# yangfei1223/CRFConv

Measured on AMD Instinct MI355X. Metric: M points/sec fwd+bwd, S3DIS 40960-pt cloud, K=16, 3 CRF iters; mIoU parity, higher is better.
Workload: dtype f32; 1 GPU; BASELINE configs[1]: S3DIS-like synthetic clouds (one point per 4 cm voxel of an 8x8x3 m box), 4 clouds x 40960 pts per GPU, K=16, ratios [4,4,4,4,2], PointConvBig(in=6, classes=13, use_crf, steps=3), train mode: fwd + weighted CE + bwd + flat-bucket grad all-reduce + SGD(momentum) step; tables resident in HBM; point order from the device collate: morton; global_batch=4, points_per_cloud=40960, parallelism=dp1 (batch-sharded)

## Files before the change

### crfconv_amd/csrc/pointconv_wide.hip

```cpp
#include "common.hpp"
#include "gridsync.hpp"

namespace crf {

using f32x4w = __attribute__((ext_vector_type(4))) float;
#ifndef WP_BLOCK_
#define WP_BLOCK_ 512
#endif
constexpr int WP_BLOCK = WP_BLOCK_, WP_WAVES = WP_BLOCK / WAVE, WP_MAX = 8;

struct WideJobs {
    const float* x[WP_MAX]; const float* gout[WP_MAX]; const float* pos_src[WP_MAX]; const float* pos_tgt[WP_MAX];
    const int32_t* idx[WP_MAX];
    const float* A1[WP_MAX]; const float* b1[WP_MAX]; const float* W2[WP_MAX]; const float* ca[WP_MAX]; const float* cb[WP_MAX];
    const float* cc[WP_MAX];
    float* dw2_partial[WP_MAX]; double* a1_partial[WP_MAX];
    int m_tgt[WP_MAX], nblk[WP_MAX], d[WP_MAX];
    float slope[WP_MAX];
    int blk_base[WP_MAX + 1];
    int njobs;
};

template <int D>
constexpr int wide_params_lds_floats() {
    return D * (D + 4) + 4 * D + 3 * D + WP_WAVES * 16 * (D + 4) + WP_WAVES * 16 * (D + 16) + 4 * WP_WAVES * 16;
}
template <int D>
__device__ __forceinline__ void wide_params_body(const WideJobs& t, const int job, const int blk, float* __restrict__ lds) {
    constexpr int T16 = D / 16, S4 = D / 4, LDW = D + 4, LDG = D + 4, LDH = D + 16, K = 16;
    constexpr int UNR = S4 > 16 ? 4 : S4;
    float* const s_w2 = lds;
    float4* const s_a1 = reinterpret_cast<float4*>(s_w2 + D * LDW);
    float* const s_coef = reinterpret_cast<float*>(s_a1 + D);
    float (*s_g)[K * LDG] = reinterpret_cast<float (*)[K * LDG]>(s_coef + 3 * D);
    float (*s_h)[K * LDH] = reinterpret_cast<float (*)[K * LDH]>(s_coef + 3 * D + WP_WAVES * K * LDG);
    float4 (*s_rel)[K] = reinterpret_cast<float4 (*)[K]>(s_coef + 3 * D + WP_WAVES * K * (LDG + LDH));
    float* s_red = s_w2;
    const int nblk = t.nblk[job], m = t.m_tgt[job];
    const float* __restrict__ x = t.x[job];
    const float* __restrict__ gout = t.gout[job];
    const float* __restrict__ pos_src = t.pos_src[job];
    const float* __restrict__ pos_tgt = t.pos_tgt[job];
    const int32_t* __restrict__ idx = t.idx[job];
    const float slope = t.slope[job];
    {
        const float* __restrict__ W2 = t.W2[job];
        for (int i = threadIdx.x; i < D * D; i += WP_BLOCK) s_w2[(i / D) * LDW + (i % D)] = W2[i];
        const float* __restrict__ A1 = t.A1[job];
        const float* __restrict__ b1 = t.b1[job];
        for (int c = threadIdx.x; c < D; c += WP_BLOCK) {
            s_a1[c] = make_float4(A1[3 * c], A1[3 * c + 1], A1[3 * c + 2], b1[c]);
            s_coef[c] = t.ca[job][c];
            s_coef[D + c] = t.cb[job][c];
            s_coef[2 * D + c] = t.cc[job][c];
        }
    }
    __syncthreads();
    const int lane = threadIdx.x & 63, wave = threadIdx.x >> 6;
    const int e = lane & 15, kq = lane >> 4;
    float* tg = s_g[wave];
    float* th = s_h[wave];
    float4* trel = s_rel[wave];
    f32x4w accW[T16][T16];
#pragma unroll
    for (int a = 0; a < T16; ++a)
#pragma unroll
        for (int b = 0; b < T16; ++b) accW[a][b] = f32x4w{0.f, 0.f, 0.f, 0.f};
    float a1acc[T16][4];
#pragma unroll
    for (int a = 0; a < T16; ++a)
#pragma unroll
        for (int b = 0; b < 4; ++b) a1acc[a][b] = 0.f;

    const int per = (m + nblk - 1) / nblk;
    const int p0 = blk * per, p1 = p0 + per < m ? p0 + per : m;
    for (int p = p0 + wave; p < p1; p += WP_WAVES) {
        const int jraw = idx[(int64_t)p * K + e];
        const bool live = jraw >= 0;
        const int64_t j = live ? jraw : 0;
        const float rx = pos_tgt[3 * (int64_t)p] - pos_src[3 * j], ry = pos_tgt[3 * (int64_t)p + 1] - pos_src[3 * j + 1],
                    rz = pos_tgt[3 * (int64_t)p + 2] - pos_src[3 * j + 2];
        int jr[4];
        bool lr[4];
#pragma unroll
        for (int r = 0; r < 4; ++r) {
            jr[r] = __shfl((int)j, 4 * kq + r, WAVE);
            lr[r] = __shfl(live ? 1 : 0, 4 * kq + r, WAVE) != 0;
        }
        constexpr bool PRELOAD = D <= 64;
        [[maybe_unused]] float xv[PRELOAD ? T16 : 1][4], gi[PRELOAD ? T16 : 1];
        if constexpr (PRELOAD) {
#pragma unroll
            for (int tj = 0; tj < T16; ++tj) {
                gi[tj] = gout[(int64_t)p * D + 16 * tj + e];
#pragma unroll
                for (int r = 0; r < 4; ++r) xv[tj][r] = x[(int64_t)jr[r] * D + 16 * tj + e];
            }
        }
        if (kq == 0) trel[e] = live ? make_float4(rx, ry, rz, 1.f) : make_float4(0.f, 0.f, 0.f, 0.f);
        f32x4w acc[T16];
#pragma unroll
        for (int tj = 0; tj < T16; ++tj) acc[tj] = f32x4w{0.f, 0.f, 0.f, 0.f};
#pragma unroll UNR
        for (int s = 0; s < S4; ++s) {
            const float4 a = s_a1[4 * s + kq];
            const float pre = fmaf(a.x, rx, fmaf(a.y, ry, fmaf(a.z, rz, a.w)));
            const float h = live ? (pre > 0.f ? pre : slope * pre) : 0.f;
            th[e * LDH + 4 * s + kq] = h;
#pragma unroll
            for (int tj = 0; tj < T16; ++tj)
                acc[tj] = __builtin_amdgcn_mfma_f32_16x16x4f32(h, s_w2[(16 * tj + e) * LDW + 4 * s + kq], acc[tj], 0, 0, 0);
        }
#pragma unroll
        for (int tj = 0; tj < T16; ++tj) {
            const int c = 16 * tj + e;
            const float va = s_coef[c], vb = s_coef[D + c], vc = s_coef[2 * D + c];
            float gic, xc[4];
            if constexpr (PRELOAD) {
                gic = gi[tj];
#pragma unroll
                for (int r = 0; r < 4; ++r) xc[r] = xv[tj][r];
            } else {
                gic = gout[(int64_t)p * D + c];
#pragma unroll
                for (int r = 0; r < 4; ++r) xc[r] = x[(int64_t)jr[r] * D + c];
            }
#pragma unroll
            for (int r = 0; r < 4; ++r) {
                const float gh = fmaf(va, gic * xc[r], fmaf(vb, acc[tj][r], vc));
                tg[(4 * kq + r) * LDG + c] = lr[r] ? gh : 0.f;
            }
        }
        __builtin_amdgcn_wave_barrier();
#pragma unroll
        for (int tj = 0; tj < T16; ++tj) acc[tj] = f32x4w{0.f, 0.f, 0.f, 0.f};
#pragma unroll UNR
        for (int s = 0; s < S4; ++s) {
            const float a = tg[e * LDG + 4 * s + kq];
#pragma unroll
            for (int tj = 0; tj < T16; ++tj)
                acc[tj] = __builtin_amdgcn_mfma_f32_16x16x4f32(a, s_w2[(4 * s + kq) * LDW + 16 * tj + e], acc[tj], 0, 0, 0);
        }
        {
            float4 rl[4];
#pragma unroll
            for (int r = 0; r < 4; ++r) rl[r] = trel[4 * kq + r];
#pragma unroll
            for (int tj = 0; tj < T16; ++tj)
#pragma unroll
                for (int r = 0; r < 4; ++r) {
                    const float h = th[(4 * kq + r) * LDH + 16 * tj + e];
                    const float gp = acc[tj][r] * (h > 0.f ? 1.f : slope);
                    a1acc[tj][0] = fmaf(gp, rl[r].x, a1acc[tj][0]);
                    a1acc[tj][1] = fmaf(gp, rl[r].y, a1acc[tj][1]);
                    a1acc[tj][2] = fmaf(gp, rl[r].z, a1acc[tj][2]);
                    a1acc[tj][3] = fmaf(gp, rl[r].w, a1acc[tj][3]);
                }
        }
#pragma unroll
        for (int s = 0; s < 4; ++s) {
            float af[T16], bf[T16];
#pragma unroll
            for (int ti = 0; ti < T16; ++ti) {
                af[ti] = tg[(4 * s + kq) * LDG + 16 * ti + e];
                bf[ti] = th[(4 * s + kq) * LDH + 16 * ti + e];
            }
#pragma unroll
            for (int ti = 0; ti < T16; ++ti)
#pragma unroll
                for (int tj = 0; tj < T16; ++tj)
                    accW[ti][tj] = __builtin_amdgcn_mfma_f32_16x16x4f32(af[ti], bf[tj], accW[ti][tj], 0, 0, 0);
        }
        __builtin_amdgcn_wave_barrier();
    }
    __syncthreads();
    for (int w = 0; w < WP_WAVES; ++w) {
        if (wave == w) {
#pragma unroll
            for (int ti = 0; ti < T16; ++ti)
#pragma unroll
                for (int tj = 0; tj < T16; ++tj)
#pragma unroll
                    for (int r = 0; r < 4; ++r) {
                        const int o = (16 * ti + 4 * kq + r) * D + 16 * tj + e;
                        s_red[o] = (w == 0 ? 0.f : s_red[o]) + accW[ti][tj][r];
                    }
        }
        __syncthreads();
    }
    {
        float* __restrict__ out = t.dw2_partial[job] + (int64_t)blk * D * D;
        for (int i = threadIdx.x; i < D * D; i += WP_BLOCK) out[i] = s_red[i];
    }
    __syncthreads();
#pragma unroll
    for (int tj = 0; tj < T16; ++tj)
#pragma unroll
        for (int q = 0; q < 4; ++q) {
            float v = a1acc[tj][q];
            v += __shfl_xor(v, 16, WAVE);
            v += __shfl_xor(v, 32, WAVE);
            if (kq == 0) s_red[(wave * D + 16 * tj + e) * 4 + q] = v;
        }
    __syncthreads();
    {
        double* __restrict__ outd = t.a1_partial[job] + (int64_t)blk * 4 * D;
        for (int i = threadIdx.x; i < 4 * D; i += WP_BLOCK) {
            double a = 0.0;
#pragma unroll
            for (int w = 0; w < WP_WAVES; ++w) a += (double)s_red[w * 4 * D + i];
            outd[i] = a;
        }
    }
}

__global__ __launch_bounds__(WP_BLOCK) void wide_params_any_kernel(const WideJobs t) {
    __shared__ __attribute__((aligned(16))) float lds[wide_params_lds_floats<64>()];
    int job = 0;
    while (job + 1 < t.njobs && t.blk_base[job + 1] <= (int)blockIdx.x) ++job;
    const int blk = (int)blockIdx.x - t.blk_base[job];
    if (t.d[job] == 32) wide_params_body<32>(t, job, blk, lds);
    else wide_params_body<64>(t, job, blk, lds);
}

template <int D>
__global__ __launch_bounds__(WP_BLOCK) void uvstats_mfma_kernel(const float* __restrict__ x, const float* __restrict__ pos_src,
                                                                const float* __restrict__ pos_tgt, const int32_t* __restrict__ idx,
                                                                int m, int nblk, const float* __restrict__ A1,
                                                                const float* __restrict__ b1, const float* __restrict__ W2, float slope,
                                                                const float* __restrict__ mean_rel, float* __restrict__ shift_out,
                                                                float* __restrict__ U, float* __restrict__ V, float* __restrict__ partial,
                                                                unsigned* __restrict__ ticket, double* __restrict__ stats) {
    constexpr int T16 = D / 16, S4 = D / 4, LDW = D + 4, K = 16;
    constexpr int UNR = S4 > 16 ? 4 : S4;
    __shared__ __attribute__((aligned(16))) float s_w2[D * LDW];
    __shared__ float4 s_a1[D];
    __shared__ float s_shift[D];
    __shared__ float s_h0[D];
    __shared__ float s_red[WP_WAVES][2][D];
    for (int i = threadIdx.x; i < D * D; i += WP_BLOCK) s_w2[(i / D) * LDW + (i % D)] = W2[i];
    for (int c = threadIdx.x; c < D; c += WP_BLOCK) {
        const float4 a = make_float4(A1[3 * c], A1[3 * c + 1], A1[3 * c + 2], b1[c]);
        s_a1[c] = a;
        const float pre = fmaf(a.x, mean_rel[0], fmaf(a.y, mean_rel[1], fmaf(a.z, mean_rel[2], a.w)));
        s_h0[c] = pre > 0.f ? pre : slope * pre;
    }
    __syncthreads();
    for (int c = threadIdx.x; c < D; c += WP_BLOCK) {
        float a = 0.f;
        for (int cp = 0; cp < D; ++cp) a = fmaf(s_h0[cp], s_w2[c * LDW + cp], a);
        s_shift[c] = a;
        if (blockIdx.x == 0) shift_out[c] = a;
    }
    __syncthreads();
    const int lane = threadIdx.x & 63, wave = threadIdx.x >> 6;
    const int e = lane & 15, kq = lane >> 4;
    float st1[T16], st2[T16];
#pragma unroll
    for (int tj = 0; tj < T16; ++tj) st1[tj] = st2[tj] = 0.f;
    const int per = (m + nblk - 1) / nblk;
    const int p0 = (int)blockIdx.x * per, p1 = p0 + per < m ? p0 + per : m;
    for (int p = p0 + wave; p < p1; p += WP_WAVES) {
        const int jraw = idx[(int64_t)p * K + e];
        const bool live = jraw >= 0;
        const int64_t j = live ? jraw : 0;
        const float rx = pos_tgt[3 * (int64_t)p] - pos_src[3 * j], ry = pos_tgt[3 * (int64_t)p + 1] - pos_src[3 * j + 1],
                    rz = pos_tgt[3 * (int64_t)p + 2] - pos_src[3 * j + 2];
        int jr[4];
        float lv[4];
#pragma unroll
        for (int r = 0; r < 4; ++r) {
            jr[r] = __shfl((int)j, 4 * kq + r, WAVE);
            lv[r] = __shfl(live ? 1.f : 0.f, 4 * kq + r, WAVE);
        }
        float xv[T16][4];
#pragma unroll
        for (int tj = 0; tj < T16; ++tj)
#pragma unroll
            for (int r = 0; r < 4; ++r) xv[tj][r] = x[(int64_t)jr[r] * D + 16 * tj + e] * lv[r];
        f32x4w acc[T16];
#pragma unroll
        for (int tj = 0; tj < T16; ++tj) acc[tj] = f32x4w{0.f, 0.f, 0.f, 0.f};
#pragma unroll UNR
        for (int s = 0; s < S4; ++s) {
            const float4 a = s_a1[4 * s + kq];
            const float pre = fmaf(a.x, rx, fmaf(a.y, ry, fmaf(a.z, rz, a.w)));
            const float h = pre > 0.f ? pre : slope * pre;
#pragma unroll
            for (int tj = 0; tj < T16; ++tj)
                acc[tj] = __builtin_amdgcn_mfma_f32_16x16x4f32(h, s_w2[(16 * tj + e) * LDW + 4 * s + kq], acc[tj], 0, 0, 0);
        }
#pragma unroll
        for (int tj = 0; tj < T16; ++tj) {
            const float sh = s_shift[16 * tj + e];
            float u = 0.f, v = 0.f;
#pragma unroll
            for (int r = 0; r < 4; ++r) {
                const float dlt = (acc[tj][r] - sh) * lv[r];
                st1[tj] += dlt;
                st2[tj] = fmaf(dlt, dlt, st2[tj]);
                u = fmaf(dlt, xv[tj][r], u);
                v += xv[tj][r];
            }
            u += __shfl_xor(u, 16, WAVE); u += __shfl_xor(u, 32, WAVE);
            v += __shfl_xor(v, 16, WAVE); v += __shfl_xor(v, 32, WAVE);
            if (kq == 0) {
                U[(int64_t)p * D + 16 * tj + e] = u;
                V[(int64_t)p * D + 16 * tj + e] = v;
            }
        }
    }
#pragma unroll
    for (int tj = 0; tj < T16; ++tj) {
        float a = st1[tj], b = st2[tj];
        a += __shfl_xor(a, 16, WAVE); a += __shfl_xor(a, 32, WAVE);
        b += __shfl_xor(b, 16, WAVE); b += __shfl_xor(b, 32, WAVE);
        if (kq == 0) { s_red[wave][0][16 * tj + e] = a; s_red[wave][1][16 * tj + e] = b; }
    }
    __syncthreads();
    const __amdgpu_buffer_rsrc_t pr = make_rsrc(partial, (int)gridDim.x * 2 * D * 4);
    for (int i = threadIdx.x; i < 2 * D; i += WP_BLOCK) {
        float a = 0.f;
#pragma unroll
        for (int w = 0; w < WP_WAVES; ++w) a += s_red[w][i / D][i % D];
        st1_sc1(pr, ((int)blockIdx.x * 2 * D + i) * 4, a);
    }
    constexpr bool ALIAS = sizeof(float) * D * LDW >= sizeof(double) * 4 * WP_BLOCK;
    __shared__ double s_own[ALIAS ? 1 : 4 * WP_BLOCK], s_tot[2 * D];
    __shared__ int s_flag;
    if (ticket == nullptr || !last_workgroup(ticket, gridDim.x, &s_flag)) return;
    double* s_buf = ALIAS ? reinterpret_cast<double*>(s_w2) : s_own;
    sum_partial_rows_f64<WP_BLOCK>(pr, (int)gridDim.x, 2 * D, s_buf, s_tot);
    if (threadIdx.x < 2 * D) stats[threadIdx.x] = s_tot[threadIdx.x];
}

#ifndef WP_PPW_BIG_
#define WP_PPW_BIG_ 3
#endif
#ifndef WP_PPW_MID_
#define WP_PPW_MID_ 3
#endif
#ifndef WP_PPW_SMALL_
#define WP_PPW_SMALL_ 1
#endif
static int64_t wide_points_per_wave(int64_t m_tgt) {
    return m_tgt >= 8192 ? WP_PPW_BIG_ : (m_tgt >= 2048 ? WP_PPW_MID_ : WP_PPW_SMALL_);
}

bool uvstats_mfma_ok(int K, int d) { return K == 16 && (d == 32 || d == 64 || d == 128); }
int uvstats_mfma_launch(const float* x, const float* pos_src, const float* pos_tgt, const int32_t* idx32, int64_t m_tgt, int d,
                        const float* A1, const float* b1, const float* W2, float slope, const float* mean_rel3, float* shift, float* U,
                        float* V, float* partial, int64_t max_blocks, int64_t* nblk_out, unsigned* ticket, double* stats, hipStream_t st) {
    int64_t nb = cdiv(m_tgt, wide_points_per_wave(m_tgt) * WP_WAVES);
    if (nb > max_blocks) nb = max_blocks;
    if (nb < 1) nb = 1;
    *nblk_out = nb;
    if (d == 32) hipLaunchKernelGGL(uvstats_mfma_kernel<32>, dim3((unsigned)nb), dim3(WP_BLOCK), 0, st, x, pos_src, pos_tgt, idx32, (int)m_tgt, (int)nb, A1, b1, W2, slope, mean_rel3, shift, U, V, partial, ticket, stats);
    else if (d == 64) hipLaunchKernelGGL(uvstats_mfma_kernel<64>, dim3((unsigned)nb), dim3(WP_BLOCK), 0, st, x, pos_src, pos_tgt, idx32, (int)m_tgt, (int)nb, A1, b1, W2, slope, mean_rel3, shift, U, V, partial, ticket, stats);
    else hipLaunchKernelGGL(uvstats_mfma_kernel<128>, dim3((unsigned)nb), dim3(WP_BLOCK), 0, st, x, pos_src, pos_tgt, idx32, (int)m_tgt, (int)nb, A1, b1, W2, slope, mean_rel3, shift, U, V, partial, ticket, stats);
    CRF_LAUNCH_CHECK();
    return CRF_OK;
}

static int64_t wide_nblk(int64_t m_tgt, int d) {
    (void)d;
    int64_t nb = cdiv(m_tgt, wide_points_per_wave(m_tgt) * WP_WAVES);
    if (nb < 1) nb = 1;
    if (nb > 2048) nb = 2048;
    return nb;
}

}

using namespace crf;

extern "C" int crfconv_pointconv_wide_params_supported(int64_t m_tgt, int K, int d) {
    return (K == 16 && (d == 32 || d == 64) && m_tgt > 0 && m_tgt < ((int64_t)1 << 27)) ? 1 : 0;
}

extern "C" int64_t crfconv_pointconv_wide_params_nblk(int64_t m_tgt, int d) {
    return m_tgt > 0 ? wide_nblk(m_tgt, d) : 0;
}

extern "C" int crfconv_pointconv_wide_params_jobs(const crf_pc_wide_job* jobs, int njobs, crf_stream_t stream) {
    CRF_REQUIRE(jobs || njobs == 0, CRF_ERR_ARG, "null pointer");
    CRF_REQUIRE(njobs >= 0, CRF_ERR_ARG, "njobs=%d < 0", njobs);
    hipStream_t st = as_stream(stream);
    for (int j = 0; j < njobs; ++j) {
        const crf_pc_wide_job& jb = jobs[j];
        CRF_REQUIRE(crfconv_pointconv_wide_params_supported(jb.m_tgt, jb.K, jb.d) == 1, CRF_ERR_UNSUPPORTED,
                    "job %d: K=%d d=%d m_tgt=%lld outside the matrix-pipe parameter pass (K = 16, d in {32, 64})", j, jb.K, jb.d,
                    (long long)jb.m_tgt);
        CRF_REQUIRE(jb.x && jb.gout && jb.pos_src && jb.pos_tgt && jb.idx32 && jb.A1 && jb.b1 && jb.W2 && jb.ca && jb.cb && jb.cc &&
                        jb.dw2_partial && jb.a1_partial, CRF_ERR_ARG, "job %d: null pointer", j);
    }
    int order[2] = {64, 32};
    int idx[64];
    int nidx = 0;
    for (int w = 0; w < 2; ++w)
        for (int j = 0; j < njobs && nidx < 64; ++j)
            if (jobs[j].d == order[w]) idx[nidx++] = j;
    CRF_REQUIRE(nidx == njobs, CRF_ERR_UNSUPPORTED, "at most 64 jobs per call");
    for (int j0 = 0; j0 < nidx; j0 += WP_MAX) {
        WideJobs t;
        const int n = nidx - j0 < WP_MAX ? nidx - j0 : WP_MAX;
        int64_t blocks = 0;
        for (int k = 0; k < n; ++k) {
            const crf_pc_wide_job& jb = jobs[idx[j0 + k]];
            t.x[k] = jb.x; t.gout[k] = jb.gout; t.pos_src[k] = jb.pos_src; t.pos_tgt[k] = jb.pos_tgt; t.idx[k] = jb.idx32;
            t.A1[k] = jb.A1; t.b1[k] = jb.b1; t.W2[k] = jb.W2; t.ca[k] = jb.ca; t.cb[k] = jb.cb; t.cc[k] = jb.cc;
            t.dw2_partial[k] = jb.dw2_partial; t.a1_partial[k] = jb.a1_partial;
            t.m_tgt[k] = (int)jb.m_tgt; t.nblk[k] = (int)wide_nblk(jb.m_tgt, jb.d); t.slope[k] = jb.slope; t.d[k] = jb.d;
            t.blk_base[k] = (int)blocks;
            blocks += t.nblk[k];
        }
        for (int k = n; k <= WP_MAX; ++k) t.blk_base[k] = (int)blocks;
        for (int k = n; k < WP_MAX; ++k) {
            t.x[k] = t.gout[k] = t.pos_src[k] = t.pos_tgt[k] = t.A1[k] = t.b1[k] = t.W2[k] = t.ca[k] = t.cb[k] = t.cc[k] = nullptr;
            t.idx[k] = nullptr; t.dw2_partial[k] = nullptr; t.a1_partial[k] = nullptr; t.m_tgt[k] = 0; t.nblk[k] = 1; t.slope[k] = 1.f; t.d[k] = 32;
        }
        t.njobs = n;
        hipLaunchKernelGGL(wide_params_any_kernel, dim3((unsigned)blocks), dim3(WP_BLOCK), 0, st, t);
        CRF_LAUNCH_CHECK();
    }
    return CRF_OK;
}
```

### crfconv_amd/ops/_base.py

```python
import ctypes

import torch

from .. import _lib
from ..graph import NeighborTable, ptr, require_gpu, stream_ptr

BN_EPS = 1e-5


def _f32c(t):
    if t.dtype is torch.float32 and t.is_contiguous():
        return t.detach()
    return t.detach().to(torch.float32).contiguous()


def _pad_channels(t, C):
    if t.shape[-1] == C:
        return t
    return torch.nn.functional.pad(t, (0, C - t.shape[-1]))


def _next_supported(c, choices):
    for v in choices:
        if c <= v:
            return v
    raise _lib.CrfConvError('channel count %d exceeds the largest supported (%d)' % (c, choices[-1]))


def _ptr_array(tensors):
    return (ctypes.c_void_p * len(tensors))(*[None if t is None else t.data_ptr() for t in tensors])



_TICKETS = {}
_raw_stream = getattr(torch._C, '_cuda_getCurrentRawStream', None)


def _stream_key(device):
    idx = device.index if isinstance(device, torch.device) else None
    if idx is None:
        dev = torch.device(device)
        idx = dev.index if dev.index is not None else torch.cuda.current_device()
    if torch.cuda.is_current_stream_capturing():
        return idx, 'capture'
    if _raw_stream is not None:
        return idx, int(_raw_stream(idx))
    return idx, int(torch.cuda.current_stream(idx).cuda_stream)


def _stream_buf(table, device, make):
    key = _stream_key(device)
    buf = table.get(key)
    if buf is None:
        buf = table[key] = make()
        if key[1] != 'capture' and (key[0], 'capture') not in table:
            table[(key[0], 'capture')] = make()
    return buf


def _ticket(device):
    return _stream_buf(_TICKETS, device, lambda: torch.zeros(_lib.load().crfconv_ticket_bytes() // 4, dtype=torch.int32, device=device))




def _pc_ticket(device):
    return ptr(_ticket(device))




def _mlp_ticket(device):
    return ptr(_ticket(device))


_sync_ws = {}


def gridsync_ws(dev):
    return _stream_buf(_sync_ws, dev, lambda: torch.zeros(_lib.load().crfconv_gridsync_workspace() // 4, dtype=torch.int32, device=dev))




def fail_word_ptrs(dev):
    want = torch.device(dev).index
    if want is None:
        want = torch.cuda.current_device()
    word = _lib.load().crfconv_gridsync_fail_word()
    keys = [k for k in _sync_ws if k[0] == want]
    first = [k for k in ((want, 'capture'), (want, int(torch.cuda.current_stream(want).cuda_stream))) if k in _sync_ws]
    rest = [k for k in reversed(keys) if k not in first]
    if len(first) + len(rest) > 8:
        import warnings
        warnings.warn('fail_word_ptrs: %d barrier workspaces on device %d, the update guard watches 8 (capture buffer, current stream, '
                      'newest streams); ops.check_gridsync() reads all of them' % (len(first) + len(rest), want))
    return [_sync_ws[k].data_ptr() + 4 * word for k in (first + rest)[:8]]


def check_gridsync(dev=None, reduced_flag=None):
    word = _lib.load().crfconv_gridsync_fail_word()
    bad = []
    want = None if dev is None else torch.device(dev).index
    for table in (_sync_ws,):
        for key, ws in list(table.items()):
            if want is not None and key[0] is not None and key[0] != want:
                continue
            code = int(ws[word].item())
            if code != 0:
                ws.zero_()
                bad.append((key, code))
    remote = False
    if reduced_flag is not None and reduced_flag.numel():
        v = float(reduced_flag.reshape(-1)[0].item())
        remote = not (v == 0.0)
        if remote:
            reduced_flag.zero_()
    if bad or remote:
        state.small_mlp_disabled = True
        where = ('device(s) %s (code 0x%x)' % (sorted({k[0] for k, _ in bad}), bad[0][1])) if bad else 'another rank of the process group'
        raise _lib.CrfConvError('grid barrier timed out on %s: a one-launch kernel could not get all its '
                                'workgroups resident; its outputs were poisoned with NaN.  The one-launch MLP path is now '
                                'disabled for this process (CRFCONV_NO_ONE_LAUNCH_MLP=1 does the same up front).' % where)




def _env_families(name):
    v = __import__('os').environ.get(name)
    if v is None:
        return False
    v = v.strip().lower()
    return True if v in ('', '1', 'all') else frozenset(q.strip() for q in v.split(',') if q.strip())


class _State:
    no_join = False
    no_fork = False
    no_prefold = False
    no_graph_tables = False
    no_mask_fold = __import__('os').environ.get('CRFCONV_NO_MASK_FOLD') is not None
    no_combine_fold = _env_families('CRFCONV_NO_COMBINE_FOLD')
    small_mlp_disabled = __import__('os').environ.get('CRFCONV_NO_ONE_LAUNCH_MLP') is not None
    small_bwd_one_launch = __import__('os').environ.get('CRFCONV_SMALL_BWD_TWO_LAUNCHES') is None
    dw_hosts_mats = __import__('os').environ.get('CRFCONV_NO_TAIL_RIDERS') is None
    mfma_min_rows = 12288
    mf_block = __import__('os').environ.get('CRFCONV_MF_BLOCK', 'auto')
    mf_block_min_rows = 65536
    mf_block_min_locality = 0.6


state = _State()
```

### crfconv_amd/ops/defer.py

```python
import ctypes

import torch

from .. import _lib
from ..graph import ptr, stream_ptr
from ._base import state

_DEFER = {'on': False, 'jobs': [], 'partials': [], 'red64': [], 'pc_wide': [], 'tn': [], 'late_calls': [], 'late_mats': [], 'folds': [], 'mlpdw': [], 'armed': False,
          'claimed': set()}


class deferred_weight_grads:

    def __init__(self, enabled=True, sink=None):
        self.enabled = enabled
        self.sink = sink

    def __enter__(self):
        self.prev = _DEFER['on']
        self.prev_sink = _DEFER.get('sink')
        _DEFER['on'] = bool(self.enabled)
        _DEFER['sink'] = self.sink
        if not self.prev:
            _DEFER['jobs'], _DEFER['folds'], _DEFER['mlpdw'], _DEFER['armed'], _DEFER['claimed'] = [], [], [], False, set()
            for k in ('partials', 'red64', 'pc_wide', 'tn', 'late_calls', 'late_mats'):
                _DEFER[k] = []
        return self

    def __exit__(self, exc_type, *exc):
        _DEFER['on'] = self.prev
        _DEFER['sink'] = self.prev_sink
        if exc_type is not None and not self.prev:
            _DEFER['jobs'], _DEFER['folds'], _DEFER['mlpdw'], _DEFER['armed'], _DEFER['claimed'] = [], [], [], False, set()
            for k in ('partials', 'red64', 'pc_wide', 'tn', 'late_calls', 'late_mats'):
                _DEFER[k] = []
        return False


def _defer_ok(params):
    W, b = params
    return (_DEFER['on'] and isinstance(W, torch.nn.Parameter) and W.is_leaf and W.requires_grad
            and (b is None or (isinstance(b, torch.nn.Parameter) and b.is_leaf)))


def _param_out(prm, shape, dev):
    sink = _DEFER.get('sink') if _DEFER['on'] else None
    if (sink is not None and isinstance(prm, torch.nn.Parameter) and prm.is_leaf and prm.requires_grad and prm.grad is None
            and prm.dtype == torch.float32 and id(prm) not in _DEFER['claimed']):
        dst = sink(prm)
        if dst is not None and dst.dtype == torch.float32 and dst.is_contiguous() and dst.numel() == prm.numel():
            _DEFER['claimed'].add(id(prm))
            return dst.view(shape), True
    return torch.empty(shape, dtype=torch.float32, device=dev), False


def _param_ret(prm, buf, direct):
    if direct:
        prm.grad = buf.view_as(prm)
        return None
    return buf


_WGRAD_BATCH_ROWS = 65536


def _defer_weight_grad(g, x, params, has_bias):
    m, Co = g.shape
    Ci = x.shape[1]
    lib = _lib.load()
    nbytes = lib.crfconv_linear_wgrad_workspace(m, Co, Ci)
    ws = torch.empty(nbytes, dtype=torch.uint8, device=g.device)
    want_b = bool(has_bias and params[1].requires_grad)
    if m <= _WGRAD_BATCH_ROWS:
        g, x = g.contiguous(), x.contiguous()
        _DEFER['partials'].append((_lib.WgradJob(g.data_ptr(), x.data_ptr(), m, Co, Ci, 1 if want_b else 0, ws.data_ptr(), nbytes), (g, x)))
        nblk = lib.crfconv_linear_wgrad_nblk(m, Co, Ci)
    else:
        nb = ctypes.c_int(0)
        _lib.call('crfconv_linear_wgrad_partial', ptr(g), ptr(x), m, Co, Ci, 1 if want_b else 0, ptr(ws), nbytes,
                  ctypes.byref(nb), stream_ptr())
        nblk = nb.value
    _DEFER['jobs'].append((params[0], params[1] if want_b else None, ws, nblk, Co, Ci))
    _arm_flush()


def _defer_tn(A, B, out):
    m, ca = A.shape
    cb = B.shape[1]
    lib = _lib.load()
    nbytes = lib.crfconv_linear_wgrad_workspace(m, ca, cb)
    ws = torch.empty(nbytes, dtype=torch.uint8, device=A.device)
    A, B = A.contiguous(), B.contiguous()
    _DEFER['partials'].append((_lib.WgradJob(A.data_ptr(), B.data_ptr(), m, ca, cb, 0, ws.data_ptr(), nbytes), (A, B)))
    _DEFER['tn'].append((ws, lib.crfconv_linear_wgrad_nblk(m, ca, cb), ca * cb, out))
    _arm_flush()


def _arm_flush():
    if not _DEFER['armed']:
        _DEFER['armed'] = True
        torch.autograd.Variable._execution_engine.queue_callback(_flush_weight_grads)


def _defer_fold1_bwd(job, keep, installs):
    _DEFER['folds'].append((job, keep, installs))
    _arm_flush()


def _mlp_dw_ret(deferred, prm, dW, direct, ws, m, ci, co, coef):
    if not deferred:
        return _param_ret(prm, dW, direct)
    _DEFER['mlpdw'].append((_lib.MlpDwJob(ws.data_ptr(), coef.data_ptr(), dW.data_ptr(), m, ci, co), (ws, coef), (prm, dW, direct)))
    _arm_flush()
    return None


def _mlp_param_outs(prm, W, dev):
    co = W.shape[0]
    outs = [_param_out(prm[0], tuple(W.shape), dev), _param_out(prm[1], (co,), dev), _param_out(prm[2], (co,), dev)]
    return outs, _defer_ok((prm[0], None))


def _mlp_param_rets(prm, outs, deferred, ws, m, ci, co, coef):
    (dW, kW), (dgamma, kg), (dbeta, kb) = outs
    return (_mlp_dw_ret(deferred, prm[0], dW, kW, ws, m, ci, co, coef), _param_ret(prm[1], dgamma, kg),
            _param_ret(prm[2], dbeta, kb))


def _install_grad(prm, gr, direct):
    gr = gr.view_as(prm)
    if prm.grad is None:
        prm.grad = gr
    elif direct:
        if prm.grad.data_ptr() != gr.data_ptr():
            gr.add_(prm.grad)
            prm.grad = gr
    else:
        prm.grad.add_(gr)


def _flush_mlp_dw():
    jobs, _DEFER['mlpdw'] = _DEFER['mlpdw'], []
    mats, _DEFER['late_mats'] = _DEFER.get('late_mats', []), []
    st = stream_ptr()
    if jobs:
        table = (_lib.MlpDwJob * len(jobs))(*[j[0] for j in jobs])
        if mats and state.dw_hosts_mats:
            arguments, install, _ = mats.pop(0)
            arrays, keep = arguments()
            _lib.call('crfconv_mlp_dw_jobs_hosting', table, len(jobs), *arrays, st)
            del keep
            install()
        else:
            _lib.call('crfconv_mlp_dw_jobs', table, len(jobs), st)
        for _, _, (prm, gr, direct) in jobs:
            _install_grad(prm, gr, direct)
    for arguments, install, _ in mats:
        arrays, keep = arguments()
        _lib.call('crfconv_crf_matrices_backward_batched', *arrays, st)
        del keep
        install()


def _defer_reduce64(partial_ptr, is_float, nblk, nslots, out, keep):
    _DEFER['red64'].append((_lib.Reduce64Job(partial_ptr, 1 if is_float else 0, int(nblk), int(nslots), out.data_ptr()), (out,) + tuple(keep)))
    _arm_flush()


def _take_red64():
    red, _DEFER['red64'] = _DEFER.get('red64', []), []
    if not red:
        return None, 0, None
    return (_lib.Reduce64Job * len(red))(*[j for j, _ in red]), len(red), red


def _flush_fold1_bwd():
    folds, _DEFER['folds'] = _DEFER['folds'], []
    if not folds:
        return
    table = (_lib.Fold1BwdJob * len(folds))(*[f[0] for f in folds])
    _lib.call('crfconv_pointconv_fold1_bwd_batched', table, len(folds), stream_ptr())
    for _, _, installs in folds:
        for prm, gr, direct in installs:
            _install_grad(prm, gr, direct)


def _flush_pc_wide():
    wide, _DEFER['pc_wide'] = _DEFER.get('pc_wide', []), []
    if not wide:
        return
    st = stream_ptr()
    lib = _lib.load()
    mfma = [w for w in wide if lib.crfconv_pointconv_wide_params_supported(w['m_tgt'], w['K'], w['d']) == 1]
    if mfma:
        wide = [w for w in wide if not any(w is v for v in mfma)]
        jobs, keep_m = [], []
        for w in mfma:
            d, dev = w['d'], w['x'].device
            nb = int(lib.crfconv_pointconv_wide_params_nblk(w['m_tgt'], d))
            pw = torch.empty((nb, d * d), dtype=torch.float32, device=dev)
            pa = torch.empty((nb, 4 * d), dtype=torch.float64, device=dev)
            c = w['coef']
            jobs.append(_lib.PcWideJob(w['x'].data_ptr(), w['g'].data_ptr(), w['pos_src'].data_ptr(), w['pos_tgt'].data_ptr(), w['idx'].data_ptr(),
                                       w['K'], w['m_tgt'], d, w['A1'].data_ptr(), w['b1'].data_ptr(), w['W2'].data_ptr(), float(w['slope']),
                                       c[0].data_ptr(), c[1].data_ptr(), c[2].data_ptr(), pw.data_ptr(), pa.data_ptr()))
            keep_m.append((w, pw, pa, nb))
        arr = (_lib.PcWideJob * len(jobs))(*jobs)
        _lib.call('crfconv_pointconv_wide_params_jobs', arr, len(jobs), st)
        for w, pw, pa, nb in keep_m:
            d = w['d']
            _DEFER['jobs'].append((w['pW2'], None, pw, nb, d, d))
            _defer_reduce64(pa.data_ptr(), False, nb, 4 * d, w['dA1b1'], (pa, w))
        if not wide:
            return
    dumps, gemms, a1s, keep = [], [], [], []
    for w in wide:
        d, E, dev = w['d'], w['m_tgt'] * w['K'], w['x'].device
        h1 = torch.empty((E, d), dtype=torch.float32, device=dev)
        gh2 = torch.empty((E, d), dtype=torch.float32, device=dev)
        rel = torch.empty((E, 3), dtype=torch.float32, device=dev)
        gw = torch.empty((E, d), dtype=torch.float32, device=dev)
        abytes = lib.crfconv_pointconv_bwd_a1_workspace(E, d)
        aws = torch.empty(abytes, dtype=torch.uint8, device=dev)
        c = w['coef']
        dumps.append(_lib.PcDumpJob(w['x'].data_ptr(), w['g'].data_ptr(), w['pos_src'].data_ptr(), w['pos_tgt'].data_ptr(), w['idx'].data_ptr(),
                                    w['K'], w['m_tgt'], d, w['A1'].data_ptr(), w['b1'].data_ptr(), w['W2'].data_ptr(), float(w['slope']),
                                    c[0].data_ptr(), c[1].data_ptr(), c[2].data_ptr(), h1.data_ptr(), gh2.data_ptr(), rel.data_ptr()))
        gemms.append(_lib.GemmJob(gh2.data_ptr(), w['W2'].data_ptr(), gw.data_ptr(), E, d, d))
        a1s.append(_lib.PcA1Job(gw.data_ptr(), h1.data_ptr(), rel.data_ptr(), E, d, float(w['slope']), aws.data_ptr(), abytes))
        keep.append((w, h1, gh2, rel, gw, aws))
    arr = (_lib.PcDumpJob * len(dumps))(*dumps)
    _lib.call('crfconv_pointconv_bwd_dump_jobs', arr, len(dumps), st)
    for w, h1, gh2, rel, gw, aws in keep:
        _defer_weight_grad(gh2, h1, (w['pW2'], None), False)
    arr = (_lib.GemmJob * len(gemms))(*gemms)
    _lib.call('crfconv_gemm_jobs', arr, len(gemms), st)
    arr = (_lib.PcA1Job * len(a1s))(*a1s)
    _lib.call('crfconv_pointconv_bwd_a1_jobs', arr, len(a1s), st)
    for w, h1, gh2, rel, gw, aws in keep:
        d, E = w['d'], w['m_tgt'] * w['K']
        _defer_reduce64((aws.data_ptr() + 255) & ~255, False, lib.crfconv_pointconv_bwd_a1_nblk(E, d), 4 * d, w['dA1b1'], (aws, gw, h1, rel))


def _flush_weight_grads():
    _flush_pc_wide()
    jobs, _DEFER['jobs'], _DEFER['armed'] = _DEFER['jobs'], [], False
    partials, _DEFER['partials'] = _DEFER.get('partials', []), []
    if partials:
        partials.sort(key=lambda e: -(e[0].M * e[0].Co * e[0].Ci))
        arr = (_lib.WgradJob * len(partials))(*[j for j, _ in partials])
        _lib.call('crfconv_linear_wgrad_partial_jobs', arr, len(partials), stream_ptr())
    arr64, n64, keep64 = _take_red64()
    tns, _DEFER['tn'] = _DEFER.get('tn', []), []
    late_calls, _DEFER['late_calls'] = _DEFER.get('late_calls', []), []
    st = stream_ptr()
    if not jobs and not tns:
        if n64:
            _lib.call('crfconv_reduce_jobs_f64', arr64, n64, st)
        _flush_fold1_bwd()
        _flush_mlp_dw()
        for fn, _ in late_calls:
            fn()
        _DEFER['claimed'] = set()
        return
    dev = (jobs[0][2] if jobs else tns[0][0]).device
    sink = _DEFER.get('sink')

    def direct(prm):
        if sink is None or prm.grad is not None or id(prm) in _DEFER['claimed']:
            return None
        dst = sink(prm)
        if dst is None or dst.dtype != torch.float32 or not dst.is_contiguous() or dst.numel() != prm.numel():
            return None
        _DEFER['claimed'].add(id(prm))
        return dst
    targets = [(direct(W), direct(b) if b is not None else None) for W, b, _, _, _, _ in jobs]
    total = sum((Co * Ci if tw is None else 0) + (Co if (b is not None and tb is None) else 0)
                for (_, b, _, _, Co, Ci), (tw, tb) in zip(jobs, targets))
    flat = torch.empty(max(total, 1), dtype=torch.float32, device=dev)
    table = (_lib.ReduceJob * (2 * len(jobs) + len(tns)))()
    installs, n, o = [], 0, 0
    for ws_t, nblk_t, nslots_t, out_t in tns:
        table[n] = _lib.ReduceJob(ws_t.data_ptr(), out_t.data_ptr(), nblk_t, nslots_t)
        n += 1
    for (W, b, ws, nblk, Co, Ci), (tw, tb) in zip(jobs, targets):
        base = ws.data_ptr()
        dw = tw is not None
        if tw is None:
            tw = flat[o:o + Co * Ci].view(Co, Ci)
            o += Co * Ci
        table[n] = _lib.ReduceJob(base, tw.data_ptr(), nblk, Co * Ci)
        installs.append((W, tw, dw))
        n += 1
        if b is not None:
            db = tb is not None
            if tb is None:
                tb = flat[o:o + Co]
                o += Co
            table[n] = _lib.ReduceJob(base + 4 * nblk * Co * Ci, tb.data_ptr(), nblk, Co)
            installs.append((b, tb, db))
            n += 1
    _lib.call('crfconv_reduce_jobs_both', table, n, None if not n64 else arr64, n64, st)
    del keep64
    _flush_fold1_bwd()
    _flush_mlp_dw()
    for fn, _ in late_calls:
        fn()
    for prm, gr, was_direct in installs:
        _install_grad(prm, gr, was_direct)
    _DEFER['claimed'] = set()
```

Measured before the change: 45.64 M points/s.

## Route d=128 PointConv weight-net parameter gradients through wave-pair MFMA kernel

Adds a d=128 variant of the fused wide parameter-gradient pass. Each pair of waves splits the output tiles in half and shares per-point gradient and hidden tiles in LDS, accumulating dW2 and the A1/b1 partials with MFMA. Layers of width 128 previously fell back to the slower non-MFMA path. The shared kernel's static LDS buffer grows to fit the largest width, which may reduce occupancy for the d=32/64 jobs launched in the same kernel.

```diff
diff --git a/crfconv_amd/csrc/pointconv_wide.hip b/crfconv_amd/csrc/pointconv_wide.hip
--- a/crfconv_amd/csrc/pointconv_wide.hip
+++ b/crfconv_amd/csrc/pointconv_wide.hip
@@ -1,5 +1,6 @@
 #include "common.hpp"
 #include "gridsync.hpp"
+#include "wgrad_body.hpp"
 
 namespace crf {
 
@@ -214,13 +215,198 @@
     }
 }
 
+constexpr int WP_PAIRS = WP_WAVES / 2;
+template <int D>
+constexpr int wide_params_pair_lds_floats() {
+    return D * (D + 4) + 4 * D + 3 * D + WP_PAIRS * 16 * (D + 4) + WP_PAIRS * 16 * (D + 16) + 4 * WP_PAIRS * 16 + 2 * WP_PAIRS * 4 * D;
+}
+template <int D>
+__device__ __forceinline__ void wide_params_pair_body(const WideJobs& t, const int job, const int blk, float* __restrict__ lds) {
+    constexpr int T16 = D / 16, TH = T16 / 2, S4 = D / 4, LDW = D + 4, LDG = D + 4, LDH = D + 16, K = 16;
+    constexpr int UNR = 4;
+    static_assert(T16 % 2 == 0, "tile halves");
+    float* const s_w2 = lds;
+    float4* const s_a1 = reinterpret_cast<float4*>(s_w2 + D * LDW);
+    float* const s_coef = reinterpret_cast<float*>(s_a1 + D);
+    float (*s_g)[K * LDG] = reinterpret_cast<float (*)[K * LDG]>(s_coef + 3 * D);
+    float (*s_h)[K * LDH] = reinterpret_cast<float (*)[K * LDH]>(s_coef + 3 * D + WP_PAIRS * K * LDG);
+    float4 (*s_rel)[K] = reinterpret_cast<float4 (*)[K]>(s_coef + 3 * D + WP_PAIRS * K * (LDG + LDH));
+    double (*s_sum)[4 * D] = reinterpret_cast<double (*)[4 * D]>(s_coef + 3 * D + WP_PAIRS * K * (LDG + LDH) + 4 * WP_PAIRS * K);
+    float* s_red = s_w2;
+    const int nblk = t.nblk[job], m = t.m_tgt[job];
+    const float* __restrict__ x = t.x[job];
+    const float* __restrict__ gout = t.gout[job];
+    const float* __restrict__ pos_src = t.pos_src[job];
+    const float* __restrict__ pos_tgt = t.pos_tgt[job];
+    const int32_t* __restrict__ idx = t.idx[job];
+    const float slope = t.slope[job];
+    {
+        for (int i = threadIdx.x; i < WP_PAIRS * 4 * D; i += WP_BLOCK) s_sum[0][i] = 0.0;
+        const float* __restrict__ W2 = t.W2[job];
+        if ((reinterpret_cast<uintptr_t>(W2) & 15) == 0) {
+            for (int i = threadIdx.x; i < D * D / 4; i += WP_BLOCK)
+                *reinterpret_cast<float4*>(s_w2 + (i / (D / 4)) * LDW + 4 * (i % (D / 4))) = reinterpret_cast<const float4*>(W2)[i];
+        } else {
+            for (int i = threadIdx.x; i < D * D; i += WP_BLOCK) s_w2[(i / D) * LDW + (i % D)] = W2[i];
+        }
+        const float* __restrict__ A1 = t.A1[job];
+        const float* __restrict__ b1 = t.b1[job];
+        for (int c = threadIdx.x; c < D; c += WP_BLOCK) {
+            s_a1[c] = make_float4(A1[3 * c], A1[3 * c + 1], A1[3 * c + 2], b1[c]);
+            s_coef[c] = t.ca[job][c];
+            s_coef[D + c] = t.cb[job][c];
+            s_coef[2 * D + c] = t.cc[job][c];
+        }
+    }
+    __syncthreads();
+    const int lane = threadIdx.x & 63, wave = threadIdx.x >> 6, pair = wave >> 1, half = wave & 1;
+    const int e = lane & 15, kq = lane >> 4;
+    const int t0 = TH * half;
+    float* tg = s_g[pair];
+    float* th = s_h[pair];
+    float4* trel = s_rel[pair];
+    f32x4w accW[TH][T16];
+#pragma unroll
+    for (int a = 0; a < TH; ++a)
+#pragma unroll
+        for (int b = 0; b < T16; ++b) accW[a][b] = f32x4w{0.f, 0.f, 0.f, 0.f};
+
+    const int per = (m + nblk - 1) / nblk;
+    const int p0 = blk * per, p1 = p0 + per < m ? p0 + per : m;
+    for (int pb = p0; pb < p1; pb += WP_PAIRS) {
+        const bool active = pb + pair < p1;
+        const int p = active ? pb + pair : p0;
+        const int jraw = idx[(int64_t)p * K + e];
+        const bool live = active && jraw >= 0;
+        const int64_t j = live ? jraw : 0;
+        const float rx = pos_tgt[3 * (int64_t)p] - pos_src[3 * j], ry = pos_tgt[3 * (int64_t)p + 1] - pos_src[3 * j + 1],
+                    rz = pos_tgt[3 * (int64_t)p + 2] - pos_src[3 * j + 2];
+        int jr[4];
+        bool lr[4];
+#pragma unroll
+        for (int r = 0; r < 4; ++r) {
+            jr[r] = __shfl((int)j, 4 * kq + r, WAVE);
+            lr[r] = __shfl(live ? 1 : 0, 4 * kq + r, WAVE) != 0;
+        }
+        if (half == 0 && kq == 0) trel[e] = live ? make_float4(rx, ry, rz, 1.f) : make_float4(0.f, 0.f, 0.f, 0.f);
+        f32x4w acc[TH];
+#pragma unroll
+        for (int tj = 0; tj < TH; ++tj) acc[tj] = f32x4w{0.f, 0.f, 0.f, 0.f};
+#pragma unroll UNR
+        for (int s = 0; s < S4; ++s) {
+            const float4 a = s_a1[4 * s + kq];
+            const float pre = fmaf(a.x, rx, fmaf(a.y, ry, fmaf(a.z, rz, a.w)));
+            const float h = live ? (pre > 0.f ? pre : slope * pre) : 0.f;
+            if ((s >= S4 / 2) == (half != 0)) th[e * LDH + 4 * s + kq] = h;
+#pragma unroll
+            for (int tj = 0; tj < TH; ++tj)
+                acc[tj] = __builtin_amdgcn_mfma_f32_16x16x4f32(h, s_w2[(16 * (t0 + tj) + e) * LDW + 4 * s + kq], acc[tj], 0, 0, 0);
+        }
+#pragma unroll
+        for (int tj = 0; tj < TH; ++tj) {
+            const int c = 16 * (t0 + tj) + e;
+            const float va = s_coef[c], vb = s_coef[D + c], vc = s_coef[2 * D + c];
+            const float gic = gout[(int64_t)p * D + c];
+            float xc[4];
+#pragma unroll
+            for (int r = 0; r < 4; ++r) xc[r] = x[(int64_t)jr[r] * D + c];
+#pragma unroll
+            for (int r = 0; r < 4; ++r) {
+                const float gh = fmaf(va, gic * xc[r], fmaf(vb, acc[tj][r], vc));
+                tg[(4 * kq + r) * LDG + c] = lr[r] ? gh : 0.f;
+            }
+        }
+        __syncthreads();
+#pragma unroll
+        for (int tj = 0; tj < TH; ++tj) acc[tj] = f32x4w{0.f, 0.f, 0.f, 0.f};
+#pragma unroll 2
+        for (int s = 0; s < D / 16; ++s) {
+            const float4 a4 = *reinterpret_cast<const float4*>(tg + e * LDG + 16 * s + 4 * kq);
+            const float av[4] = {a4.x, a4.y, a4.z, a4.w};
+#pragma unroll
+            for (int ee = 0; ee < 4; ++ee)
+#pragma unroll
+                for (int tj = 0; tj < TH; ++tj)
+                    acc[tj] = __builtin_amdgcn_mfma_f32_16x16x4f32(av[ee], s_w2[(16 * s + 4 * kq + ee) * LDW + 16 * (t0 + tj) + e], acc[tj], 0, 0, 0);
+        }
+        {
+            float4 rl[4];
+#pragma unroll
+            for (int r = 0; r < 4; ++r) rl[r] = trel[4 * kq + r];
+#pragma unroll
+            for (int tj = 0; tj < TH; ++tj) {
+                double v[4] = {0.0, 0.0, 0.0, 0.0};
+#pragma unroll
+                for (int r = 0; r < 4; ++r) {
+                    const float h = th[(4 * kq + r) * LDH + 16 * (t0 + tj) + e];
+                    const double gp = (double)(acc[tj][r] * (h > 0.f ? 1.f : slope));
+                    v[0] += gp * (double)rl[r].x; v[1] += gp * (double)rl[r].y; v[2] += gp * (double)rl[r].z; v[3] += gp * (double)rl[r].w;
+                }
+#pragma unroll
+                for (int c = 0; c < 4; ++c) {
+                    v[c] += __shfl_xor(v[c], 16, WAVE);
+                    v[c] += __shfl_xor(v[c], 32, WAVE);
+                }
+                if (kq == 0) {
+                    double* const dst = &s_sum[pair][4 * (16 * (t0 + tj) + e)];
+#pragma unroll
+                    for (int c = 0; c < 4; ++c) dst[c] += v[c];
+                }
+            }
+        }
+#pragma unroll 2
+        for (int s = 0; s < 4; ++s) {
+            float af[TH], bf[T16];
+#pragma unroll
+            for (int ti = 0; ti < TH; ++ti) af[ti] = tg[(4 * s + kq) * LDG + 16 * (t0 + ti) + e];
+#pragma unroll
+            for (int tj = 0; tj < T16; ++tj) bf[tj] = th[(4 * s + kq) * LDH + 16 * tj + e];
+#pragma unroll
+            for (int ti = 0; ti < TH; ++ti)
+#pragma unroll
+                for (int tj = 0; tj < T16; ++tj)
+                    accW[ti][tj] = __builtin_amdgcn_mfma_f32_16x16x4f32(af[ti], bf[tj], accW[ti][tj], 0, 0, 0);
+        }
+        __syncthreads();
+    }
+    for (int q = 0; q < WP_PAIRS; ++q) {
+        if (pair == q) {
+#pragma unroll
+            for (int ti = 0; ti < TH; ++ti)
+#pragma unroll
+                for (int tj = 0; tj < T16; ++tj)
+#pragma unroll
+                    for (int r = 0; r < 4; ++r) {
+                        const int o = (16 * (t0 + ti) + 4 * kq + r) * LDW + 16 * tj + e;
+                        s_red[o] = (q == 0 ? 0.f : s_red[o]) + accW[ti][tj][r];
+                    }
+        }
+        __syncthreads();
+    }
+    {
+        float* __restrict__ out = t.dw2_partial[job] + (int64_t)blk * D * D;
+        for (int i = threadIdx.x; i < D * D; i += WP_BLOCK) out[i] = s_red[(i / D) * LDW + (i % D)];
+    }
+    {
+        double* __restrict__ outd = t.a1_partial[job] + (int64_t)blk * 4 * D;
+        for (int i = threadIdx.x; i < 4 * D; i += WP_BLOCK) {
+            double a = 0.0;
+#pragma unroll
+            for (int w = 0; w < WP_PAIRS; ++w) a += s_sum[w][i];
+            outd[i] = a;
+        }
+    }
+}
+
 __global__ __launch_bounds__(WP_BLOCK) void wide_params_any_kernel(const WideJobs t) {
-    __shared__ __attribute__((aligned(16))) float lds[wide_params_lds_floats<64>()];
+    __shared__ __attribute__((aligned(16))) float lds[wide_params_pair_lds_floats<128>()];
+    static_assert(wide_params_pair_lds_floats<128>() >= wide_params_lds_floats<64>(), "the buffer of the largest width");
     int job = 0;
     while (job + 1 < t.njobs && t.blk_base[job + 1] <= (int)blockIdx.x) ++job;
     const int blk = (int)blockIdx.x - t.blk_base[job];
     if (t.d[job] == 32) wide_params_body<32>(t, job, blk, lds);
-    else wide_params_body<64>(t, job, blk, lds);
+    else if (t.d[job] == 64) wide_params_body<64>(t, job, blk, lds);
+    else wide_params_pair_body<128>(t, job, blk, lds);
 }
 
 template <int D>
@@ -363,8 +549,7 @@
 }
 
 static int64_t wide_nblk(int64_t m_tgt, int d) {
-    (void)d;
-    int64_t nb = cdiv(m_tgt, wide_points_per_wave(m_tgt) * WP_WAVES);
+    int64_t nb = d == 128 ? wg_plan(m_tgt * 16, 128, 128).nblk : cdiv(m_tgt, wide_points_per_wave(m_tgt) * WP_WAVES);
     if (nb < 1) nb = 1;
     if (nb > 2048) nb = 2048;
     return nb;
@@ -375,7 +560,7 @@
 using namespace crf;
 
 extern "C" int crfconv_pointconv_wide_params_supported(int64_t m_tgt, int K, int d) {
-    return (K == 16 && (d == 32 || d == 64) && m_tgt > 0 && m_tgt < ((int64_t)1 << 27)) ? 1 : 0;
+    return (K == 16 && (d == 32 || d == 64 || d == 128) && m_tgt > 0 && m_tgt < ((int64_t)1 << 27)) ? 1 : 0;
 }
 
 extern "C" int64_t crfconv_pointconv_wide_params_nblk(int64_t m_tgt, int d) {
@@ -389,15 +574,15 @@
     for (int j = 0; j < njobs; ++j) {
         const crf_pc_wide_job& jb = jobs[j];
         CRF_REQUIRE(crfconv_pointconv_wide_params_supported(jb.m_tgt, jb.K, jb.d) == 1, CRF_ERR_UNSUPPORTED,
-                    "job %d: K=%d d=%d m_tgt=%lld outside the matrix-pipe parameter pass (K = 16, d in {32, 64})", j, jb.K, jb.d,
+                    "job %d: K=%d d=%d m_tgt=%lld outside the matrix-pipe parameter pass (K = 16, d in {32, 64, 128})", j, jb.K, jb.d,
                     (long long)jb.m_tgt);
         CRF_REQUIRE(jb.x && jb.gout && jb.pos_src && jb.pos_tgt && jb.idx32 && jb.A1 && jb.b1 && jb.W2 && jb.ca && jb.cb && jb.cc &&
                         jb.dw2_partial && jb.a1_partial, CRF_ERR_ARG, "job %d: null pointer", j);
     }
-    int order[2] = {64, 32};
+    int order[3] = {128, 64, 32};
     int idx[64];
     int nidx = 0;
-    for (int w = 0; w < 2; ++w)
+    for (int w = 0; w < 3; ++w)
         for (int j = 0; j < njobs && nidx < 64; ++j)
             if (jobs[j].d == order[w]) idx[nidx++] = j;
     CRF_REQUIRE(nidx == njobs, CRF_ERR_UNSUPPORTED, "at most 64 jobs per call");
diff --git a/crfconv_amd/ops/_base.py b/crfconv_amd/ops/_base.py
--- a/crfconv_amd/ops/_base.py
+++ b/crfconv_amd/ops/_base.py
@@ -144,6 +144,7 @@
     small_mlp_disabled = __import__('os').environ.get('CRFCONV_NO_ONE_LAUNCH_MLP') is not None
     small_bwd_one_launch = __import__('os').environ.get('CRFCONV_SMALL_BWD_TWO_LAUNCHES') is None
     dw_hosts_mats = __import__('os').environ.get('CRFCONV_NO_TAIL_RIDERS') is None
+    no_wide128 = __import__('os').environ.get('CRFCONV_NO_WIDE128') is not None
     mfma_min_rows = 12288
     mf_block = __import__('os').environ.get('CRFCONV_MF_BLOCK', 'auto')
     mf_block_min_rows = 65536
diff --git a/crfconv_amd/ops/defer.py b/crfconv_amd/ops/defer.py
--- a/crfconv_amd/ops/defer.py
+++ b/crfconv_amd/ops/defer.py
@@ -191,7 +191,8 @@
         return
     st = stream_ptr()
     lib = _lib.load()
-    mfma = [w for w in wide if lib.crfconv_pointconv_wide_params_supported(w['m_tgt'], w['K'], w['d']) == 1]
+    mfma = [w for w in wide if lib.crfconv_pointconv_wide_params_supported(w['m_tgt'], w['K'], w['d']) == 1
+            and not (state.no_wide128 and w['d'] == 128)]
     if mfma:
         wide = [w for w in wide if not any(w is v for v in mfma)]
         jobs, keep_m = [], []
```

Measured after the change: 46.13 M points/s (median of 6 runs). +1.1%, better.
